# ielym/fastvision

Measured on AMD Instinct MI355X. Metric: images/sec (640×640, bs=32/GPU) YOLOv3 train step, 1/2/4/8 MI355X, higher is better.
Workload: dtype bf16

## Files before the change

### fastvision_amd/_lib.py

```python
import ctypes as C
import os

HERE = os.path.dirname(os.path.abspath(__file__))
LIB_PATH = os.path.join(HERE, 'csrc', 'libfastvision_amd.so')
if os.environ.get('FVA_LIB_PATH'):
    if os.environ.get('FVA_EXPERIMENTS') == '1':
        LIB_PATH = os.environ['FVA_LIB_PATH']
        import sys
        print(f'fastvision_amd: EXPERIMENT -- loading {LIB_PATH} instead of the in-tree library (FVA_LIB_PATH)', file=sys.stderr)
    else:
        raise RuntimeError('fastvision_amd: FVA_LIB_PATH is set but FVA_EXPERIMENTS=1 is not -- refusing to load another library silently')

F32, BF16 = 0, 1


class ConvDesc(C.Structure):
    _fields_ = [(n, C.c_int32) for n in ('dtype', 'B', 'H', 'W', 'Cin', 'Cout', 'ksize', 'stride', 'in_pad', 'dy_pad')]


class HeadLevel(C.Structure):
    _fields_ = [('data', C.c_void_p), ('grad', C.c_void_p),
                ('sb', C.c_int64), ('sa', C.c_int64), ('sy', C.c_int64), ('sx', C.c_int64), ('sk', C.c_int64),
                ('B', C.c_int32), ('A', C.c_int32), ('H', C.c_int32), ('W', C.c_int32), ('K', C.c_int32),
                ('anchor_w', C.c_float * 8), ('anchor_h', C.c_float * 8), ('stride', C.c_float)]
# ... 41 lines not shown

_P, _I, _L, _F = C.c_void_p, C.c_int32, C.c_int64, C.c_float
_D = C.POINTER(ConvDesc)
_H = C.POINTER(HeadLevel)

PROTOTYPES = {
    'fva_last_error': (C.c_char_p, []),
    'fva_version': (_I, []),
    'fva_profile_start': (_I, [_I]),
    'fva_profile_classes': (_I, [C.c_uint32, _I]),
    'fva_side_stream_fork': (_I, [_P, C.POINTER(C.c_void_p)]),
    'fva_side_stream_join': (_I, [_P]),
    'fva_side_stream_renew': (_I, []),
    'fva_conv_debug_stamps': (_I, [_P, _I]),
    'fva_conv_patch_kernel': (_I, [_I]),
    'fva_profile_stop': (_I, [_P, _P, _P, _I]),
    'fva_conv_pack_weights': (_I, [_D, _P, _P, _P, _P]),
    'fva_conv_packed_elems': (_L, [_D, _I]),
    'fva_conv_pack_weights_multi': (_I, [_P, _I, _L, _P]),
    'fva_conv_pack_weights_tiled': (_I, [_P, _I, _I, _P]),
    'fva_conv_last_kernel': (C.c_char_p, []),
    'fva_conv_fwd': (_I, [_D, _P, _P, _P, _P, _P]),
    'fva_conv1x1_fwd_apply': (_I, [_D, _P, _P, _P, _P, _I, _P, _P, _P, _P, _P]),
    'fva_conv_fwd_acc': (_I, [_D, _P, _P, _P, _P, _I, _P]),
    'fva_bn_acc_finalize': (_I, [C.POINTER(BnFwdAcc), _L, _I, _P]),
    'fva_bn_silu_apply_acc': (_I, [_I, _P, C.POINTER(BnFwdAcc), _P, _I, _P, _I, _I, _I, _I, _I, _P]),
    'fva_conv1x1_fwd_apply_acc': (_I, [_D, _P, C.POINTER(BnFwdAcc), _P, _I, _P, _P, _P, _P, _I, _P]),
    'fva_conv_fwd_bnact': (_I, [_D, _P, _P, _P, _P, _P, _P, _I, _P]),
    'fva_conv_stat_blocks': (_I, [_D]),
    'fva_conv_dgrad': (_I, [_D, _P, _P, _P, _P, _P]),
# ... 75 lines not shown
    'fva_softmax_ce_workspace': (_L, [_I]),
    'fva_softmax_ce': (_I, [_P, _P, _I, _P, _I, _I, _I, _P, _P, _P, _P]),
    'fva_top1_accuracy': (_I, [_P, _I, _P, _I, _I, _I, _P, _P, _P]),
    'fva_bn_relu_apply': (_I, [_I, _P, _P, _P, _P, _I, _I, _I, _I, _I, _P]),
    'fva_bn_relu_bwd_reduce': (_I, [_I, _P, _P, _P, _P, _P, _P, _P, _I, _L, _I, _P]),
    'fva_bn_relu_bwd_apply': (_I, [_I, _P, _P, _P, _P, _P, _P, _P, _P, _I, _I, _I, _I, _I, _P]),
    'fva_bn_bias_running_mean': (_I, [_I, _P, _P, _F, _P]),
    'fva_bn_eval_coeffs_bias': (_I, [_I, _P, _P, _P, _P, _P, _F, _P, _P, _P]),
    'fva_adaptive_avgpool7_fwd': (_I, [_I, _P, _I, _I, _I, _I, _I, _P, _P]),
    'fva_adaptive_avgpool7_bwd': (_I, [_I, _P, _I, _I, _I, _I, _P, _P]),
    'fva_dropout_fwd': (_I, [_I, _P, _P, _L, _F, _P, _P]),
    'fva_dropout_bwd': (_I, [_I, _P, _P, _P, _L, _F, _P]),
}
LABEL_I64, LABEL_F32 = 0, 1
REDUCE_MEAN, REDUCE_SUM = 0, 1
UNCHECKED = {'fva_conv_patch_kernel', 'fva_sgd_chunk_elems', 'fva_rows_relu_bwd_rows', 'fva_colour_workspace', 'fva_conv_dgrad_stat_rows', 'fva_bias_relu_bwd_rows', 'fva_colsum_scratch_rows', 'fva_last_error', 'fva_version', 'fva_profile_stop', 'fva_conv_last_kernel', 'fva_conv_packed_elems', 'fva_conv_stat_blocks', 'fva_conv_wgrad_workspace', 'fva_conv_wgrad_plan',
             'fva_stem_stat_blocks', 'fva_stem_fused_blocks', 'fva_stem_wgrad_workspace', 'fva_stem_fwd_workspace', 'fva_stem_wgrad_mfma_workspace', 'fva_bn_bwd_blocks', 'fva_bn_partial_rows', 'fva_yolov3_loss_workspace',
             'fva_demo_loss_workspace', 'fva_nms_candidates_workspace', 'fva_nms_select_workspace', 'fva_softmax_ce_workspace'}

_lib = None


def load():
    global _lib
    if _lib is not None:
        return _lib
    if not os.path.exists(LIB_PATH):
        raise RuntimeError(f'fastvision_amd: {LIB_PATH} is missing -- the HIP extension is REQUIRED (no CPU fallback). '
                           'Build it with `python fastvision_amd/csrc/build.py`.')
    lib = C.CDLL(LIB_PATH)
    for name, (res, args) in PROTOTYPES.items():
# ... 30 lines not shown
```

### fastvision_amd/csrc/conv_igemm.hip

```cpp
#include <stddef.h>
#include <stdlib.h>

#include "common.h"

namespace {

enum { EPI_STATS = 0, EPI_PLAIN = 1, EPI_HEAD = 2, EPI_BNACT = 3, EPI_BNB = 4 };
constexpr int MAX_TAPS = 10;

struct IgemmParams {
    const void* in;
    const void* wt;
    void* out;
    float* stats;
    int acc_rep, bnb_rep, ax_rep;
    long long* stats_acc;
    const float* bias;
    const float* scale;
    int act;
    const float* shift;
    int M, N, C;
    int OW, OHW;
    FastDiv div_ow, div_ohw;
    int in_img, in_row;
// ... 17 lines not shown
    const float *ax_scale, *ax_shift;
    int ax_pad, ax_res_pad, ax_H, ax_W;
    long long* ax_acc;
    long long* ax_zero;
    const float *ax_gamma, *ax_beta;
    float *ax_rm, *ax_rv;
    long long* ax_nbt;
    float ax_momentum, ax_eps;
    BnN ax_n;
    float *ax_save_mean, *ax_save_rstd, *ax_scale_out, *ax_shift_out;
    long long* stamps;
    int stamp_rows;
    int pt_tx, pt_ty, pt_H, pt_W;
    int pt_tiles, pt_tpb;
    FastDiv pt_div_tx, pt_div_img;
};

struct BnbCoef {
    float sc[8], sh[8], mu[8], rs[8];
};
__device__ __forceinline__ void bnb_load(const IgemmParams& p, int n, BnbCoef& k) {
#pragma unroll
    for (int e = 0; e < 8; ++e) {
        int c = n + e;
        c = c < p.N ? c : p.N - 1;
        c = c >= p.bnb_C ? c - p.bnb_C : c;
        k.sc[e] = p.bnb_scale[c]; k.sh[e] = p.bnb_shift[c]; k.mu[e] = p.bnb_mean[c]; k.rs[e] = p.bnb_rstd[c];
    }
}
template <int BN, int NT>
__device__ __forceinline__ float bnb_coef_at(const IgemmParams& p, int i, int n0) {
// ... 169 lines not shown
__device__ __forceinline__ void foreach_acc(Acc<float>& acc, int lane, F&& f) {
    const int r = lane & 31, h = lane >> 5;
#pragma unroll
    for (int mt = 0; mt < 2; ++mt)
#pragma unroll
        for (int nt = 0; nt < 2; ++nt)
#pragma unroll
            for (int e = 0; e < 16; ++e) f(mt * 32 + (e & 3) + 8 * (e >> 2) + 4 * h, nt * 32 + r, nt, acc.a[mt][nt][e]);
}

template <int N>
__device__ __forceinline__ void wait_vmcnt() {
    asm volatile("s_waitcnt vmcnt(%0)" ::"n"(N) : "memory");
}

template <typename T, int BM, int BN, int EPI, int NSTAGE, bool AX = false>
__global__ __launch_bounds__((BM / 64) * (BN / 64) * 64) void igemm_kernel(const IgemmParams p) {
    static_assert(!AX || (sizeof(T) == 2 && EPI == EPI_STATS), "the produced-operand form is the bf16 training forward of a 1x1 layer");
    constexpr int EPC = 16 / (int)sizeof(T);
    constexpr int BK = 8 * EPC;
    constexpr int WN = BN / 64;
    constexpr int NW = (BM / 64) * WN;
    constexpr int NT = NW * 64;
    static_assert(NW % 2 == 0, "the source swizzle assumes an even wave count");
    constexpr int A_BYTES = BM * 128, B_BYTES = BN * 128, STAGE = A_BYTES + B_BYTES;
    constexpr int A_ITERS = BM / (8 * NW), B_ITERS = BN / (8 * NW);
    constexpr bool IS_BF16 = sizeof(T) == 2;
    extern __shared__ __attribute__((aligned(16))) char smem[];

    const int tid = threadIdx.x, lane = tid & 63, w = tid >> 6;
    const int wr = w / WN, wc = w % WN;
    auto stamp = [&](int i) {
        if (p.stamps && tid == 0 && (int)blockIdx.x < p.stamp_rows) p.stamps[(int64_t)blockIdx.x * 8 + i] = wall_clock64();
    };
    stamp(0);

    const int nwg = gridDim.x, bid = blockIdx.x;
    const int xcd = bid & 7, xq = nwg >> 3, xr = nwg & 7;
    const int logical = (xcd < xr ? xcd * (xq + 1) : xr * (xq + 1) + (xcd - xr) * xq) + (bid >> 3);
    const int mblk = logical / p.nblocks, nblk = logical - mblk * p.nblocks;
    const int m0 = mblk * BM, n0 = nblk * BN;

    const T* a_ptr[A_ITERS];
    const T* b_ptr[B_ITERS];
    const int lrow = lane >> 3;
    const int sw = ((w & 1) << 2) + (lane >> 4);
    const int chunk = (lane & 7) ^ sw;
    const int tapsel = chunk >> 2;
    const int sub = p.halfrow ? (chunk & 3) : chunk;
#pragma unroll
    for (int i = 0; i < A_ITERS; ++i) {
        int m = m0 + (i * NW + w) * 8 + lrow;
        m = m < p.M ? m : p.M - 1;
        const uint32_t b = fd_div((uint32_t)m, p.div_ohw);
        const uint32_t rem = (uint32_t)m - b * (uint32_t)p.OHW;
        const uint32_t oy = fd_div(rem, p.div_ow);
// ... 7 lines not shown
        n = n < p.N ? n : p.N - 1;
        b_ptr[i] = (const T*)p.wt + (int64_t)n * p.C + sub * EPC;
    }

    constexpr bool USE_KTAB = BN >= 128;
    constexpr int COEF_BYTES = (EPI == EPI_BNB && IS_BF16 && BN >= 128) ? 4 * BN * 4 : 0;
    float* coef_tab = (float*)(smem + NSTAGE * STAGE);
    int* ktab = (int*)(smem + NSTAGE * STAGE + COEF_BYTES);
    constexpr int COEF_PER_THREAD = COEF_BYTES > 0 ? 4 * BN / NT : 0;
    float coef_v[COEF_PER_THREAD > 0 ? COEF_PER_THREAD : 1];
    if constexpr (COEF_BYTES > 0) {
#pragma unroll
        for (int j = 0; j < COEF_PER_THREAD; ++j) coef_v[j] = bnb_coef_at<BN, NT>(p, tid + j * NT, n0);
    }
    if constexpr (USE_KTAB) {
        const int nent = p.halfrow ? 2 * p.ktiles : p.ktiles;
        for (int e = tid; e < nent; e += NT) {
            int t, kk;
            if (p.halfrow) { t = e; kk = 0; }
            else if (p.ktaps) { kk = e / p.ktaps; t = e - kk * p.ktaps; }
            else { t = e / p.kt_per_tap; kk = e - t * p.kt_per_tap; }
            int tp = 0, tw = 0;
#pragma unroll
            for (int i = 0; i < MAX_TAPS; ++i)
                if (i == t) { tp = p.tap_pix[i]; tw = p.tap_w[i]; }
            ktab[2 * e] = tp * p.C + kk * BK;
            ktab[2 * e + 1] = tw * p.N * p.C + kk * BK;
        }
        __syncthreads();
    }
    stamp(6);
    int ld_tap = 0, ld_kk = 0;
    auto load_tile = [&](int kt, int stage) {
        char* sA = smem + stage * STAGE;
        char* sB = sA + A_BYTES;
        int aoff, boff;
        if constexpr (USE_KTAB) {
            const int e = p.halfrow ? 2 * kt + tapsel : kt;
            aoff = ktab[2 * e];
            boff = ktab[2 * e + 1];
// ... 22 lines not shown
        constexpr int CPR = BN / 8, RSTEP = NT / CPR;
        static_assert(BM * CPR / NT == 8, "the prefetch covers the whole store loop");
        const int cc = tid % CPR, r0 = tid / CPR;
        const int n = n0 + cc * 8;
#pragma unroll
        for (int j = 0; j < 8; ++j) {
            const int m = m0 + r0 + j * RSTEP;
            int64_t oi = 0;
            if (n < p.N && m < p.M) {
                int64_t pixel = m;
                if (!p.out_dense) {
                    const uint32_t b = fd_div((uint32_t)m, p.div_ohw);
                    const uint32_t rem = (uint32_t)m - b * (uint32_t)p.OHW;
                    const uint32_t oy = fd_div(rem, p.div_ow);
                    const uint32_t ox = rem - oy * (uint32_t)p.OW;
                    pixel = (int64_t)b * p.out_img + (int64_t)(oy * p.osy + p.ooy) * p.out_row + (ox * p.osx + p.oox);
                }
                oi = pixel * p.out_pitch + n;
            }
            if constexpr (EPI == EPI_BNB) y_pre[j] = ld_stream((const bf16_t*)p.bnb_y + oi);
            if (p.addend != nullptr) a_pre[j] = ld_stream((const bf16_t*)p.addend + oi);
        }
    }

    Acc<T> acc;
    if constexpr (sizeof(T) == 2) {
#pragma unroll
        for (int i = 0; i < 4; ++i)
#pragma unroll
            for (int j = 0; j < 4; ++j) acc.a[i][j] = f32x4{0.f, 0.f, 0.f, 0.f};
    } else {
// ... 147 lines not shown
            ax_fl[i] = (live ? 1u : 0u) | (zp > 0 && live ? ((ox == 0 ? 2u : 0u) | (ox == (uint32_t)p.ax_W - 1 ? 4u : 0u) | (oy == 0 ? 8u : 0u) |
                                                           (oy == (uint32_t)p.ax_H - 1 ? 16u : 0u)) : 0u);
        }
        ax_load_raw(0, std::integral_constant<int, 0>{});
        if constexpr (AXT) {
            for (int c = tid; c < p.C; c += NT) ax_coef(c, logical == 0, ax_tab[c], ax_tab[p.C + c]);
            __syncthreads();
        }
        if (AXT && p.ax_acc != nullptr && logical == 0) {
            if (tid == 0 && p.ax_nbt) *p.ax_nbt += 1;
            fx_zero(p.ax_zero, p.C, p.ax_rep, tid, NT);
        }
        ax_issue_b(0, 0);
    } else {
        load_tile(0, 0);
        if (p.ktiles > 1) load_tile(1, 1);
    }
    stamp(1);
    for (int kt = 0; kt < p.ktiles; ++kt) {
        if constexpr (AX) {
            if (AXS == 1 || (kt & 1) == 0) ax_step(kt, std::integral_constant<int, 0>{});
            else ax_step(kt, std::integral_constant<int, AXS - 1>{});
            if (kt == 0) stamp(2);
        } else {
        if (kt == 0 && p.ktiles > 1) wait_vmcnt<LPT>();
        else wait_vmcnt<0>();
        __builtin_amdgcn_s_barrier();
        if (kt == 0) stamp(2);
        if (kt >= 1 && kt + 1 < p.ktiles) load_tile(kt + 1, st_cur ^ 1);
        }
        const char* sA = smem + st_cur * STAGE;
        const char* sB = sA + A_BYTES;
        st_cur ^= 1;
        if constexpr (IS_BF16) {
            const int r = lane & 15, g = lane >> 4, sr = (r >> 1) & 7;
            const char* pa = sA + (wr * 64 + r) * 128;
            const char* pb = sB + (wc * 64 + r) * 128;
#pragma unroll
            for (int ks = 0; ks < 2; ++ks) {
                const int co = ((ks * 4 + g) ^ sr) << 4;
                bf16x8 af[4], bfr[4];
#pragma unroll
                for (int t = 0; t < 4; ++t) {
                    af[t] = *(const bf16x8*)(pa + t * 16 * 128 + co);
// ... 111 lines not shown
                        if (p.stats_acc != nullptr) fx_atomic_add(fx_replica(p.stats_acc, p.N, p.acc_rep), p.N, which, n0 + col, s);
                        else *(p.stats + ((int64_t)mblk * 2 + which) * p.N + n0 + col) = s;
                    }
                }
                __syncthreads();
            }
        }
    }

    auto out_pixel = [&](int m) -> int64_t {
        if (p.out_dense) return m;
        const uint32_t b = fd_div((uint32_t)m, p.div_ohw);
        const uint32_t rem = (uint32_t)m - b * (uint32_t)p.OHW;
        const uint32_t oy = fd_div(rem, p.div_ow);
        const uint32_t ox = rem - oy * (uint32_t)p.OW;
        return (int64_t)b * p.out_img + (int64_t)(oy * p.osy + p.ooy) * p.out_row + (ox * p.osx + p.oox);
    };

    if constexpr (EPI == EPI_HEAD) {
        float* out = (float*)p.out;
        foreach_acc(acc, lane, [&](int row, int col, int, float v) {
            const int m = m0 + wrow0 + row, n = n0 + wcol0 + col;
            if (m < p.M && n < p.N) out[(int64_t)m * p.out_pitch + n] = v + p.bias[n];
        });
    } else if constexpr (!IS_BF16) {
        float* out = (float*)p.out;
        int64_t pix_cache = -1;
        int m_cache = -1;
        constexpr bool bnb = EPI == EPI_BNB;
        float b1[2] = {0.f, 0.f}, b2[2] = {0.f, 0.f}, ksc[2], ksh[2], kmu[2], krs[2];
        if constexpr (bnb) {
// ... 38 lines not shown
                    if (lane < 32) {
                        red[(0 * WMc + wr) * BN + wcol0 + i * 32 + lane] = b1[i];
                        red[(1 * WMc + wr) * BN + wcol0 + i * 32 + lane] = b2[i];
                    }
                }
                __syncthreads();
                if (w < BN / 32) {
                    const int which = lane >> 5, col = w * 32 + (lane & 31);
                    float t = 0.f;
#pragma unroll
                    for (int k = 0; k < WMc; ++k) t += red[(which * WMc + k) * BN + col];
                    const int n = n0 + col;
                    const int sub = n >= p.bnb_C ? 1 : 0, per = p.N > p.bnb_C ? 2 : 1;
                    if (n < p.N) {
                        if (p.bnb_acc != nullptr) fx_atomic_add(fx_replica(p.bnb_acc, p.bnb_C, p.bnb_rep), p.bnb_C, which, n - sub * p.bnb_C, t);
                        else *(p.bnb_part + (((int64_t)(p.bnb_row0 + mblk) * per + sub) * 2 + which) * p.bnb_C + (n - sub * p.bnb_C)) = t;
                    }
                }
            }
        }
    } else {
        constexpr int PITCH = BN * 2 + 16;
        if constexpr (EPI == EPI_BNB && COEF_BYTES == 0) {
            coef_tab = (float*)(smem + BM * PITCH);
            static_assert(4 * BN <= NT || EPI != EPI_BNB || COEF_BYTES > 0, "one table entry per thread");
            if (tid < 4 * BN) coef_v[0] = bnb_coef_at<BN, NT>(p, tid, n0);
        }
        {
            const int r = lane & 15, g = lane >> 4;
#pragma unroll
            for (int mt = 0; mt < 4; ++mt)
// ... 1 lines not shown
                for (int nt = 0; nt < 4; ++nt) {
                    f32x4 v = acc.a[mt][nt];
                    const int col = wcol0 + nt * 16 + 4 * g;
                    if constexpr (EPI == EPI_BNACT) {
#pragma unroll
                        for (int j = 0; j < 4; ++j) v[j] = bnact_f(p, v[j], n0 + col + j < p.N ? n0 + col + j : p.N - 1);
                    }
                    *(u32x2*)(smem + (wrow0 + mt * 16 + r) * PITCH + col * 2) = u32x2{cvt_pk_bf16(v[0], v[1]), cvt_pk_bf16(v[2], v[3])};
                }
        }
        if constexpr (EPI == EPI_BNB && COEF_BYTES == 0) {
            if (tid < 4 * BN) coef_tab[tid] = coef_v[0];
        }
        __syncthreads();
        stamp(4);
        store_tile_bf16<EPI, BM, BN, NT, PITCH>(p, smem, tid, n0, mblk, [&](int row) { const int m = m0 + row; return m < p.M ? out_pixel(m) : (int64_t)-1; },
                                                EPI == EPI_BNB ? y_pre : nullptr, PREFETCH ? a_pre : nullptr, coef_tab);
    }
    if constexpr (AX) {

    }
    stamp(5);
}

template <typename T, int BM, int BN, int EPI, int NSTAGE, bool AX = false>
int launch_one(const IgemmParams& p, hipStream_t s) {
    const int mblocks = cdiv(p.M, BM);
    IgemmParams q = p;
    q.nblocks = cdiv(p.N, BN);
    static const bool stamp_tiles = [] { const char* e = getenv("FVA_STAMP_IGEMM"); return e && atoi(e) != 0; }();
    q.stamps = stamp_tiles ? fva_debug_stamps_ptr() : nullptr;
    q.stamp_rows = stamp_tiles ? fva_debug_stamps_rows() : 0;
    constexpr int KTAB_MAX = 16384;
    const int nent = (p.halfrow ? 2 : 1) * p.ktiles;
    if (BN >= 128 && nent * 8 > KTAB_MAX) return fva_fail(FVA_ERR_ARG, "igemm: %d k-tiles exceed the offset table (%d)", p.ktiles, KTAB_MAX / 8);
    const int ktab_bytes = BN >= 128 ? (nent * 8 > 4096 ? (nent * 8 + 255) & ~255 : 4096) : 0;
    constexpr int coef_bytes = (EPI == EPI_BNB && sizeof(T) == 2 && BN >= 128) ? 4 * BN * 4 : 0;
    const int smem = NSTAGE * (BM + BN) * 128 + ktab_bytes + coef_bytes;
    static bool attr_done = false;
    if (!attr_done) {
        (void)hipFuncSetAttribute((const void*)igemm_kernel<T, BM, BN, EPI, NSTAGE, AX>, hipFuncAttributeMaxDynamicSharedMemorySize,
                                  NSTAGE * (BM + BN) * 128 + (BN >= 128 ? KTAB_MAX : 0) + coef_bytes);
        attr_done = true;
    }
    hipLaunchKernelGGL((igemm_kernel<T, BM, BN, EPI, NSTAGE, AX>), dim3(mblocks * q.nblocks), dim3((BM / 64) * (BN / 64) * 64), smem, s, q);
    FVA_LAUNCH_CHECK("igemm_kernel");
    fva_note_kernel(AX ? (BM == 128 ? "igemm128ax" : "igemm256x64ax") : (BM == 128 ? "igemm128" : "igemm256x64"));
    return FVA_OK;
}

template <int CS, int BN, int NSL, int EPI>
__global__ __launch_bounds__(256, 2) void pconv_kernel(const IgemmParams p) {
    constexpr int TH = 8, TW = 32, PW = TW + 2, NPIX = (TH + 2) * PW;
    constexpr int PIXB = CS * 2;
    constexpr int CPP = PIXB / 16;
    constexpr int PPI = 1024 / PIXB;
    constexpr int PATCH_INSTR = (NPIX + PPI - 1) / PPI, PATCH_BYTES = PATCH_INSTR * 1024;
    constexpr int WSTEP_BYTES = BN * PIXB, WPW = WSTEP_BYTES / 1024 / 4;
    static_assert(WSTEP_BYTES % 4096 == 0, "whole DMA instructions per wave");
    constexpr int STEPS = 9 * NSL;
// ... 442 lines not shown
    p.pt_div_img = make_fastdiv(p.pt_tx * p.pt_ty);
    const int tiles = pdgrad2_tiles(B, H, W);
    if (p.C == 64 && p.N == 32) return launch_pdgrad2_one<64, 32, 1, EPI>(p, tiles, s);
    if (p.C == 128 && p.N == 64) return launch_pdgrad2_one<64, 64, 2, EPI>(p, tiles, s);
    return fva_fail(FVA_ERR_ARG, "pdgrad2: unsupported channels %d -> %d", p.C, p.N);
}

struct Igemm8Diag {
    long long* stamps;
    int stamp_rows;
};

#ifndef FVA_EPI_STAMPS
#define FVA_EPI_STAMPS 0
#endif
template <int EPI>
__global__ __launch_bounds__(512) void igemm8_kernel(const IgemmParams p, const Igemm8Diag sk) {
    constexpr int MT = 8;
    constexpr int WM = 16 * MT;
    constexpr int BM = 2 * WM, BN = 256, NT = 512, BK = 64;
    constexpr int HALF = 128 * 128, BUF = 4 * HALF;
    constexpr int EPI_BYTES = BM * (BN * 2 + 16);
    constexpr int TAB0 = EPI_BYTES > 2 * BUF ? EPI_BYTES : 2 * BUF;
    extern __shared__ __attribute__((aligned(16))) char smem[];
    const int tid = threadIdx.x, lane = tid & 63, w = tid >> 6;
    const int wr = w >> 2, wc = w & 3;
    auto stamp = [&](int i) {
        if (sk.stamps && tid == 0 && (int)blockIdx.x < sk.stamp_rows) {
            sk.stamps[(int64_t)blockIdx.x * 8 + i] = wall_clock64();
            sk.stamps[(int64_t)blockIdx.x * 8 + 4 + i] = clock64();
        }
    };
#if !FVA_EPI_STAMPS
    stamp(0);
#endif

    const int nwg = gridDim.x, bid = blockIdx.x;
    const int xcd = bid & 7, xq = nwg >> 3, xr = nwg & 7;
    const int logical = (xcd < xr ? xcd * (xq + 1) : xr * (xq + 1) + (xcd - xr) * xq) + (bid >> 3);
    const int KT = p.ktiles;

    int* ktab = (int*)(smem + TAB0);
    for (int e = tid; e < KT; e += NT) {
        int t, kk;
        if (p.ktaps) { kk = e / p.ktaps; t = e - kk * p.ktaps; }
        else { t = e / p.kt_per_tap; kk = e - t * p.kt_per_tap; }
        int tp = 0, tw = 0;
#pragma unroll
        for (int i = 0; i < MAX_TAPS; ++i)
            if (i == t) { tp = p.tap_pix[i]; tw = p.tap_w[i]; }
        ktab[2 * e] = tp * p.C + kk * BK;
        ktab[2 * e + 1] = tw * p.N * p.C + kk * BK;
    }

    const int lrow = lane >> 3;
    const int chunk = (lane & 7) ^ (((w & 1) << 2) + (lane >> 4));
    const int r = lane & 15, g = lane >> 4, sr = (r >> 1) & 7;
    const int co0 = (g ^ sr) << 4, co1 = ((4 + g) ^ sr) << 4;
    const int a_row = (wr * 64 + r) * 128, b_row = (wc * 32 + r) * 128;

    {
        const int tile = logical, kt0 = 0, kt1 = KT;
        const int mblk = tile / p.nblocks, nblk = tile - mblk * p.nblocks;
        const int m0 = mblk * BM, n0 = nblk * BN;
        __syncthreads();
        float* coef_tab = (float*)(smem + TAB0 + 4096);
        if constexpr (EPI == EPI_BNB) bnb_fill_lds<BN, NT>(p, coef_tab, tid, n0);

        uint32_t a_off[2][2], b_off[2][2];
#pragma unroll
        for (int h = 0; h < 2; ++h)
#pragma unroll
            for (int i = 0; i < 2; ++i) {
                const int rh = (i * 8 + w) * 8 + lrow;
                int m = m0 + (rh >> 6) * WM + h * 64 + (rh & 63);
                m = m < p.M ? m : p.M - 1;
                const uint32_t b = fd_div((uint32_t)m, p.div_ohw);
                const uint32_t rem = (uint32_t)m - b * (uint32_t)p.OHW;
                const uint32_t oy = fd_div(rem, p.div_ow);
// ... 154 lines not shown
                    if (n0 + col < p.N) {
                        if (p.stats_acc != nullptr) fx_atomic_add(fx_replica(p.stats_acc, p.N, p.acc_rep), p.N, which, n0 + col, s);
                        else *(p.stats + ((int64_t)mblk * 2 + which) * p.N + n0 + col) = s;
                    }
                }
                __syncthreads();
            }
        }

        auto out_pixel = [&](int m) -> int64_t {
            if (p.out_dense) return m;
            const uint32_t b = fd_div((uint32_t)m, p.div_ohw);
            const uint32_t rem = (uint32_t)m - b * (uint32_t)p.OHW;
            const uint32_t oy = fd_div(rem, p.div_ow);
            const uint32_t ox = rem - oy * (uint32_t)p.OW;
            return (int64_t)b * p.out_img + (int64_t)(oy * p.osy + p.ooy) * p.out_row + (ox * p.osx + p.oox);
        };
        constexpr int PITCH = BN * 2 + 16;
#if FVA_EPI_STAMPS
        stamp(1);
#endif
#pragma unroll
        for (int mi = 0; mi < MT; ++mi)
#pragma unroll
            for (int ni = 0; ni < 4; ++ni) {
                f32x4 v = acc[mi][ni];
                if constexpr (EPI == EPI_BNACT) {
#pragma unroll
                    for (int j = 0; j < 4; ++j) v[j] = bnact_f(p, v[j], n0 + col_e + ni * 16 + j);
                }
                *(u32x2*)(smem + (row_e + mi * 16) * PITCH + (col_e + ni * 16) * 2) = u32x2{cvt_pk_bf16(v[0], v[1]), cvt_pk_bf16(v[2], v[3])};
            }
        __syncthreads();
#if FVA_EPI_STAMPS
        stamp(2);
#endif
        store_tile_bf16<EPI, BM, BN, NT, PITCH>(p, smem, tid_e, n0, mblk, [&](int row) { const int m = m0 + row; return m < p.M ? out_pixel(m) : (int64_t)-1; },
                                                nullptr, nullptr, EPI == EPI_BNB ? coef_tab : nullptr);
    }
    stamp(3);
}

constexpr int IGEMM8_SMEM = 256 * (256 * 2 + 16) + 4096 + 4096;

inline bool igemm8_enabled() {
    static bool v = [] {
        const char* e = getenv("FVA_IGEMM8");
        return !e || atoi(e) != 0;
    }();
    return v;
}
inline bool use_igemm8(int dtype, int64_t M, int N, int C, int ntaps, int64_t in_pixels) {
    if (!igemm8_enabled() || dtype != FVA_BF16 || N % 256 || C % 64) return false;
    if (in_pixels * C * 2 >= (1ll << 31) || (int64_t)(ntaps + 1) * N * C * 2 >= (1ll << 31)) return false;
    const int64_t ktiles = (int64_t)ntaps * (C / 64), tiles = (int64_t)cdiv(M, 256) * (N / 256);
    if (ktiles > 496 || ktiles < 8) return false;
    if (tiles < 128) return false;
    static const int min_kt = [] { const char* e = getenv("FVA_IGEMM8_MINKT"); return e ? atoi(e) : 16; }();
    return ktiles >= min_kt || tiles <= 256;
}

long long* g_stamps = nullptr;
int g_stamp_rows = 0;

template <int EPI>
int launch_igemm8(const IgemmParams& p, hipStream_t s) {
    IgemmParams q = p;
    q.nblocks = p.N / 256;
    const int tiles = cdiv(p.M, 256) * q.nblocks;
    static bool attr_done = false;
    if (!attr_done) {
        (void)hipFuncSetAttribute((const void*)igemm8_kernel<EPI>, hipFuncAttributeMaxDynamicSharedMemorySize, IGEMM8_SMEM);
        attr_done = true;
    }
    Igemm8Diag sk{};
    sk.stamps = g_stamps;
    sk.stamp_rows = g_stamp_rows;
    hipLaunchKernelGGL((igemm8_kernel<EPI>), dim3(tiles), dim3(512), IGEMM8_SMEM, s, q, sk);
    fva_note_kernel("igemm8");
    FVA_LAUNCH_CHECK("igemm8_kernel");
    return FVA_OK;
}

inline bool wide_tile(int N) { return N >= 128; }

inline int tile_bm(int , int , int N) { return wide_tile(N) ? 128 : 256; }

template <int EPI>
int launch_igemm(int dtype, const IgemmParams& p, hipStream_t s) {
    if (dtype == FVA_BF16) {
        if constexpr (EPI != EPI_HEAD) {
            if (!p.halfrow && use_igemm8(dtype, p.M, p.N, p.C, p.ktiles / p.kt_per_tap, (int64_t)(p.M / p.OHW + 1) * p.in_img))
                return launch_igemm8<EPI>(p, s);
// ... 217 lines not shown
        }
    }
}

inline int pair_max_cin() {
    static int v = [] {
        const char* e = getenv("FVA_DGRAD_PAIR_MAX");
        return e ? atoi(e) : 64;
    }();
    return v;
}
inline bool dgrad_paired(int dtype, int ksize, int stride, int Cin, int Cout) {
    return ksize == 3 && stride == 2 && Cin <= pair_max_cin() && !use_pdgrad2(dtype, ksize, stride, Cout, Cin);
}

int packed_taps(const fva_conv_desc* d, int for_dgrad) {
    if (for_dgrad && dgrad_paired(d->dtype, d->ksize, d->stride, d->Cin, d->Cout)) return 12;

    const int kk = d->ksize * d->ksize;
    const int C = for_dgrad ? d->Cout : d->Cin;
    return (halfrow_mode(d->dtype, C) && (kk & 1)) ? kk + 1 : kk;
}

}

long long* fva_debug_stamps_ptr() { return g_stamps; }
int fva_debug_stamps_rows() { return g_stamp_rows; }
extern "C" {

int fva_conv_patch_kernel(int on) {
    const int prev = pconv_enabled() ? 1 : 0;
    g_pconv = on ? 1 : 0;
    return prev;
}

int fva_conv_debug_stamps(void* stamps, int32_t rows) {
    if (stamps && rows < 1) return fva_fail(FVA_ERR_ARG, "fva_conv_debug_stamps: rows must be >= 1");
    g_stamps = (long long*)stamps;
    g_stamp_rows = stamps ? rows : 0;
    return FVA_OK;
}

int64_t fva_conv_packed_elems(const fva_conv_desc* d, int for_dgrad) {
    if (!d) return 0;
    return (int64_t)packed_taps(d, for_dgrad) * d->Cout * d->Cin;
}

// ... 354 lines not shown
            if (rc) return rc;
            p.bnb_row0 += dgrad_launch_rows(d, p.M, p.N, p.C, nt, in_pixels);
        }
        return FVA_OK;
    }
    p.M = d->B * JH * JW;
    p.OW = JW;
    p.OHW = JH * JW;
    p.div_ow = make_fastdiv(p.OW);
    p.div_ohw = make_fastdiv(p.OHW);
    p.y0 = p.x0 = 0;
    p.out_dense = 0;
    p.out_img = d->H * d->W;
    p.out_row = d->W;
    p.osy = p.osx = 2;
    for (int py = 0; py < 2; ++py)
        for (int px = 0; px < 2; ++px) {
            int khs[2], yo[2], nky, kws[2], xo[2], nkx;
            if (py == 0) { nky = 1; khs[0] = 1; yo[0] = d->dy_pad; }
            else { nky = 2; khs[0] = 0; yo[0] = d->dy_pad + 1; khs[1] = 2; yo[1] = d->dy_pad; }
            if (px == 0) { nkx = 1; kws[0] = 1; xo[0] = d->dy_pad; }
            else { nkx = 2; kws[0] = 0; xo[0] = d->dy_pad + 1; kws[1] = 2; xo[1] = d->dy_pad; }
            int nt = 0;
            for (int a = 0; a < nky; ++a)
                for (int b = 0; b < nkx; ++b) {
                    p.tap_pix[nt] = yo[a] * p.in_row + xo[b];
                    p.tap_w[nt] = khs[a] * 3 + kws[b];
                    ++nt;
                }
            p.tap_w[nt] = 9;
            finish_taps(p, nt, d->dtype);
            p.ooy = py;
            p.oox = px;
            rc = f ? launch_igemm<EPI_BNB>(d->dtype, p, (hipStream_t)stream) : launch_igemm<EPI_PLAIN>(d->dtype, p, (hipStream_t)stream);
            if (rc) return rc;
            p.bnb_row0 += dgrad_launch_rows(d, p.M, p.N, p.C, nt, in_pixels);
        }
    return FVA_OK;
}

}
```

### include/fastvision_amd.h

```cpp
#ifndef FASTVISION_AMD_H
#define FASTVISION_AMD_H

#include <stdint.h>

#ifdef __cplusplus
extern "C" {
#endif

typedef enum { FVA_F32 = 0, FVA_BF16 = 1 } fva_dtype;

typedef enum {
    FVA_OK = 0,
    FVA_ERR_ARG = -1,
    FVA_ERR_LAUNCH = -2,
    FVA_ERR_WORKSPACE = -3
} fva_status;

const char* fva_last_error(void);
int fva_version(void);

int fva_profile_start(int32_t max_spans);
int fva_profile_classes(uint32_t mask, int32_t stride);

int fva_side_stream_fork(void* main_stream, void** side_stream);
// ... 15 lines not shown
typedef struct {
    const float* w;
    void* w_fwd;
    void* w_dgrad;
    int32_t Cout, Cin, ksize, taps_fwd, taps_dgrad, dtype;
    int32_t dgrad_paired;
    int32_t tile_start;
} fva_pack_entry;
int fva_conv_pack_weights_multi(const fva_pack_entry* table, int32_t n, int64_t max_elems, void* stream);
int fva_conv_pack_weights_tiled(const fva_pack_entry* table, int32_t n, int32_t total_tiles, void* stream);

const char* fva_conv_last_kernel(void);

int fva_conv_debug_stamps(void* stamps, int32_t rows);
int fva_conv_patch_kernel(int on);

int fva_conv_fwd(const fva_conv_desc* d, const void* x, const void* w_fwd, void* y, float* stats_partial, void* stream);
int fva_conv1x1_fwd_apply(const fva_conv_desc* d, const void* y_prev, const float* scale, const float* shift, const void* residual,
                          int32_t res_pad, void* z, const void* w_fwd, void* y, float* stats_partial, void* stream);
int fva_conv_fwd_bnact(const fva_conv_desc* d, const void* x, const void* w_fwd, const float* scale, const float* shift,
                       const void* residual, void* z, int32_t z_pad, void* stream);
int32_t fva_conv_stat_blocks(const fva_conv_desc* d);

int fva_conv_dgrad(const fva_conv_desc* d, const void* dy, const void* w_dgrad, void* dx, const void* addend, void* stream);

typedef struct {
    const void* y;
    const float *scale, *shift, *mean, *rstd;
    float* partial;
    int64_t* acc;
// ... 257 lines not shown
```

Baseline: 1123.

## Group the four stride-2 dgrad parity classes into single grouped GEMM launches

The stride-2 3x3 data-gradient conv used to run as four separate implicit-GEMM launches, one per output parity class, each with a different tap count. The classes are now packed into a per-launch table, and one grouped launch per kernel variant (igemm8 or the 128x128 tile) covers all of them, each block picking its class from its block index. This cuts launch count and the tail idle time between small launches. In exchange the params struct grows, blocks pay for class selection, and launches that mix 1-, 2- and 4-tap classes carry uneven per-block work. It is on by default and can be turned off with an env var or API toggle.

```diff
diff --git a/fastvision_amd/_lib.py b/fastvision_amd/_lib.py
--- a/fastvision_amd/_lib.py
+++ b/fastvision_amd/_lib.py
@@ -79,6 +79,7 @@
     'fva_side_stream_renew': (_I, []),
     'fva_conv_debug_stamps': (_I, [_P, _I]),
     'fva_conv_patch_kernel': (_I, [_I]),
+    'fva_conv_dgrad_grouped': (_I, [_I]),
     'fva_profile_stop': (_I, [_P, _P, _P, _I]),
     'fva_conv_pack_weights': (_I, [_D, _P, _P, _P, _P]),
     'fva_conv_packed_elems': (_L, [_D, _I]),
@@ -184,7 +185,7 @@
 }
 LABEL_I64, LABEL_F32 = 0, 1
 REDUCE_MEAN, REDUCE_SUM = 0, 1
-UNCHECKED = {'fva_conv_patch_kernel', 'fva_sgd_chunk_elems', 'fva_rows_relu_bwd_rows', 'fva_colour_workspace', 'fva_conv_dgrad_stat_rows', 'fva_bias_relu_bwd_rows', 'fva_colsum_scratch_rows', 'fva_last_error', 'fva_version', 'fva_profile_stop', 'fva_conv_last_kernel', 'fva_conv_packed_elems', 'fva_conv_stat_blocks', 'fva_conv_wgrad_workspace', 'fva_conv_wgrad_plan',
+UNCHECKED = {'fva_conv_patch_kernel', 'fva_conv_dgrad_grouped', 'fva_sgd_chunk_elems', 'fva_rows_relu_bwd_rows', 'fva_colour_workspace', 'fva_conv_dgrad_stat_rows', 'fva_bias_relu_bwd_rows', 'fva_colsum_scratch_rows', 'fva_last_error', 'fva_version', 'fva_profile_stop', 'fva_conv_last_kernel', 'fva_conv_packed_elems', 'fva_conv_stat_blocks', 'fva_conv_wgrad_workspace', 'fva_conv_wgrad_plan',
              'fva_stem_stat_blocks', 'fva_stem_fused_blocks', 'fva_stem_wgrad_workspace', 'fva_stem_fwd_workspace', 'fva_stem_wgrad_mfma_workspace', 'fva_bn_bwd_blocks', 'fva_bn_partial_rows', 'fva_yolov3_loss_workspace',
              'fva_demo_loss_workspace', 'fva_nms_candidates_workspace', 'fva_nms_select_workspace', 'fva_softmax_ce_workspace'}
 
diff --git a/fastvision_amd/csrc/conv_igemm.hip b/fastvision_amd/csrc/conv_igemm.hip
--- a/fastvision_amd/csrc/conv_igemm.hip
+++ b/fastvision_amd/csrc/conv_igemm.hip
@@ -7,6 +7,15 @@
 
 enum { EPI_STATS = 0, EPI_PLAIN = 1, EPI_HEAD = 2, EPI_BNACT = 3, EPI_BNB = 4 };
 constexpr int MAX_TAPS = 10;
+
+constexpr int GRP_CLASSES = 4, GRP_TAPS = 4;
+struct TapClass {
+    int tap_pix[GRP_TAPS], tap_w[GRP_TAPS];
+    int ntaps, ktiles;
+    int ooy, oox;
+    int bnb_row0;
+    int tile0;
+};
 
 struct IgemmParams {
     const void* in;
@@ -55,7 +64,23 @@
     int pt_tx, pt_ty, pt_H, pt_W;
     int pt_tiles, pt_tpb;
     FastDiv pt_div_tx, pt_div_img;
+    int ngrp, grp_tiles;
+    TapClass grp[GRP_CLASSES];
 };
+
+__device__ __forceinline__ TapClass grp_class(const IgemmParams& p, int logical) {
+    TapClass c = p.grp[0];
+#pragma unroll
+    for (int i = 1; i < GRP_CLASSES; ++i)
+        if (i < p.ngrp && logical >= p.grp[i].tile0) c = p.grp[i];
+    return c;
+}
+__device__ __forceinline__ void grp_tap(const TapClass& c, int t, int& tp, int& tw) {
+    tp = 0; tw = 0;
+#pragma unroll
+    for (int i = 0; i < GRP_TAPS; ++i)
+        if (i == t) { tp = c.tap_pix[i]; tw = c.tap_w[i]; }
+}
 
 struct BnbCoef {
     float sc[8], sh[8], mu[8], rs[8];
@@ -255,9 +280,10 @@
     asm volatile("s_waitcnt vmcnt(%0)" ::"n"(N) : "memory");
 }
 
-template <typename T, int BM, int BN, int EPI, int NSTAGE, bool AX = false>
+template <typename T, int BM, int BN, int EPI, int NSTAGE, bool AX = false, bool GRP = false>
 __global__ __launch_bounds__((BM / 64) * (BN / 64) * 64) void igemm_kernel(const IgemmParams p) {
     static_assert(!AX || (sizeof(T) == 2 && EPI == EPI_STATS), "the produced-operand form is the bf16 training forward of a 1x1 layer");
+    static_assert(!GRP || (!AX && BN >= 128 && (EPI == EPI_PLAIN || EPI == EPI_BNB)), "the grouped form is the stride-2 data gradient on the wide tile");
     constexpr int EPC = 16 / (int)sizeof(T);
     constexpr int BK = 8 * EPC;
     constexpr int WN = BN / 64;
@@ -276,11 +302,21 @@
     };
     stamp(0);
 
-    const int nwg = gridDim.x, bid = blockIdx.x;
+    int nwg = gridDim.x, bid = blockIdx.x;
+    TapClass cls = {};
+    if constexpr (GRP) {
+        cls = grp_class(p, bid);
+        bid -= cls.tile0;
+        nwg = p.grp_tiles;
+    }
     const int xcd = bid & 7, xq = nwg >> 3, xr = nwg & 7;
     const int logical = (xcd < xr ? xcd * (xq + 1) : xr * (xq + 1) + (xcd - xr) * xq) + (bid >> 3);
-    const int mblk = logical / p.nblocks, nblk = logical - mblk * p.nblocks;
+    const int tile = logical;
+    const int ktiles = GRP ? cls.ktiles : p.ktiles;
+    const int ooy = GRP ? cls.ooy : p.ooy, oox = GRP ? cls.oox : p.oox;
+    const int mblk = tile / p.nblocks, nblk = tile - mblk * p.nblocks;
     const int m0 = mblk * BM, n0 = nblk * BN;
+    const int srow = GRP ? cls.bnb_row0 + mblk : mblk;
 
     const T* a_ptr[A_ITERS];
     const T* b_ptr[B_ITERS];
@@ -318,16 +354,21 @@
         for (int j = 0; j < COEF_PER_THREAD; ++j) coef_v[j] = bnb_coef_at<BN, NT>(p, tid + j * NT, n0);
     }
     if constexpr (USE_KTAB) {
-        const int nent = p.halfrow ? 2 * p.ktiles : p.ktiles;
+        const int nent = (!GRP && p.halfrow) ? 2 * ktiles : ktiles;
+        const int ktaps = GRP ? (p.ktaps ? cls.ntaps : 0) : p.ktaps;
         for (int e = tid; e < nent; e += NT) {
             int t, kk;
-            if (p.halfrow) { t = e; kk = 0; }
-            else if (p.ktaps) { kk = e / p.ktaps; t = e - kk * p.ktaps; }
+            if (!GRP && p.halfrow) { t = e; kk = 0; }
+            else if (ktaps) { kk = e / ktaps; t = e - kk * ktaps; }
             else { t = e / p.kt_per_tap; kk = e - t * p.kt_per_tap; }
             int tp = 0, tw = 0;
-#pragma unroll
-            for (int i = 0; i < MAX_TAPS; ++i)
-                if (i == t) { tp = p.tap_pix[i]; tw = p.tap_w[i]; }
+            if constexpr (GRP) {
+                grp_tap(cls, t, tp, tw);
+            } else {
+#pragma unroll
+                for (int i = 0; i < MAX_TAPS; ++i)
+                    if (i == t) { tp = p.tap_pix[i]; tw = p.tap_w[i]; }
+            }
             ktab[2 * e] = tp * p.C + kk * BK;
             ktab[2 * e + 1] = tw * p.N * p.C + kk * BK;
         }
@@ -380,7 +421,7 @@
                     const uint32_t rem = (uint32_t)m - b * (uint32_t)p.OHW;
                     const uint32_t oy = fd_div(rem, p.div_ow);
                     const uint32_t ox = rem - oy * (uint32_t)p.OW;
-                    pixel = (int64_t)b * p.out_img + (int64_t)(oy * p.osy + p.ooy) * p.out_row + (ox * p.osx + p.oox);
+                    pixel = (int64_t)b * p.out_img + (int64_t)(oy * p.osy + ooy) * p.out_row + (ox * p.osx + oox);
                 }
                 oi = pixel * p.out_pitch + n;
             }
@@ -558,20 +599,20 @@
         ax_issue_b(0, 0);
     } else {
         load_tile(0, 0);
-        if (p.ktiles > 1) load_tile(1, 1);
+        if (ktiles > 1) load_tile(1, 1);
     }
     stamp(1);
-    for (int kt = 0; kt < p.ktiles; ++kt) {
+    for (int kt = 0; kt < ktiles; ++kt) {
         if constexpr (AX) {
             if (AXS == 1 || (kt & 1) == 0) ax_step(kt, std::integral_constant<int, 0>{});
             else ax_step(kt, std::integral_constant<int, AXS - 1>{});
             if (kt == 0) stamp(2);
         } else {
-        if (kt == 0 && p.ktiles > 1) wait_vmcnt<LPT>();
+        if (kt == 0 && ktiles > 1) wait_vmcnt<LPT>();
         else wait_vmcnt<0>();
         __builtin_amdgcn_s_barrier();
         if (kt == 0) stamp(2);
-        if (kt >= 1 && kt + 1 < p.ktiles) load_tile(kt + 1, st_cur ^ 1);
+        if (kt >= 1 && kt + 1 < ktiles) load_tile(kt + 1, st_cur ^ 1);
         }
         const char* sA = smem + st_cur * STAGE;
         const char* sB = sA + A_BYTES;
@@ -713,7 +754,7 @@
         const uint32_t rem = (uint32_t)m - b * (uint32_t)p.OHW;
         const uint32_t oy = fd_div(rem, p.div_ow);
         const uint32_t ox = rem - oy * (uint32_t)p.OW;
-        return (int64_t)b * p.out_img + (int64_t)(oy * p.osy + p.ooy) * p.out_row + (ox * p.osx + p.oox);
+        return (int64_t)b * p.out_img + (int64_t)(oy * p.osy + ooy) * p.out_row + (ox * p.osx + oox);
     };
 
     if constexpr (EPI == EPI_HEAD) {
@@ -782,7 +823,7 @@
                     const int sub = n >= p.bnb_C ? 1 : 0, per = p.N > p.bnb_C ? 2 : 1;
                     if (n < p.N) {
                         if (p.bnb_acc != nullptr) fx_atomic_add(fx_replica(p.bnb_acc, p.bnb_C, p.bnb_rep), p.bnb_C, which, n - sub * p.bnb_C, t);
-                        else *(p.bnb_part + (((int64_t)(p.bnb_row0 + mblk) * per + sub) * 2 + which) * p.bnb_C + (n - sub * p.bnb_C)) = t;
+                        else *(p.bnb_part + (((int64_t)(p.bnb_row0 + srow) * per + sub) * 2 + which) * p.bnb_C + (n - sub * p.bnb_C)) = t;
                     }
                 }
             }
@@ -814,7 +855,7 @@
         }
         __syncthreads();
         stamp(4);
-        store_tile_bf16<EPI, BM, BN, NT, PITCH>(p, smem, tid, n0, mblk, [&](int row) { const int m = m0 + row; return m < p.M ? out_pixel(m) : (int64_t)-1; },
+        store_tile_bf16<EPI, BM, BN, NT, PITCH>(p, smem, tid, n0, srow, [&](int row) { const int m = m0 + row; return m < p.M ? out_pixel(m) : (int64_t)-1; },
                                                 EPI == EPI_BNB ? y_pre : nullptr, PREFETCH ? a_pre : nullptr, coef_tab);
     }
     if constexpr (AX) {
@@ -823,9 +864,9 @@
     stamp(5);
 }
 
-template <typename T, int BM, int BN, int EPI, int NSTAGE, bool AX = false>
+template <typename T, int BM, int BN, int EPI, int NSTAGE, bool AX = false, bool GRP = false>
 int launch_one(const IgemmParams& p, hipStream_t s) {
-    const int mblocks = cdiv(p.M, BM);
+    const int mblocks = cdiv(p.M, BM) * (GRP ? p.ngrp : 1);
     IgemmParams q = p;
     q.nblocks = cdiv(p.N, BN);
     static const bool stamp_tiles = [] { const char* e = getenv("FVA_STAMP_IGEMM"); return e && atoi(e) != 0; }();
@@ -839,11 +880,11 @@
     const int smem = NSTAGE * (BM + BN) * 128 + ktab_bytes + coef_bytes;
     static bool attr_done = false;
     if (!attr_done) {
-        (void)hipFuncSetAttribute((const void*)igemm_kernel<T, BM, BN, EPI, NSTAGE, AX>, hipFuncAttributeMaxDynamicSharedMemorySize,
+        (void)hipFuncSetAttribute((const void*)igemm_kernel<T, BM, BN, EPI, NSTAGE, AX, GRP>, hipFuncAttributeMaxDynamicSharedMemorySize,
                                   NSTAGE * (BM + BN) * 128 + (BN >= 128 ? KTAB_MAX : 0) + coef_bytes);
         attr_done = true;
     }
-    hipLaunchKernelGGL((igemm_kernel<T, BM, BN, EPI, NSTAGE, AX>), dim3(mblocks * q.nblocks), dim3((BM / 64) * (BN / 64) * 64), smem, s, q);
+    hipLaunchKernelGGL((igemm_kernel<T, BM, BN, EPI, NSTAGE, AX, GRP>), dim3(mblocks * q.nblocks), dim3((BM / 64) * (BN / 64) * 64), smem, s, q);
     FVA_LAUNCH_CHECK("igemm_kernel");
     fva_note_kernel(AX ? (BM == 128 ? "igemm128ax" : "igemm256x64ax") : (BM == 128 ? "igemm128" : "igemm256x64"));
     return FVA_OK;
@@ -1316,8 +1357,9 @@
 #ifndef FVA_EPI_STAMPS
 #define FVA_EPI_STAMPS 0
 #endif
-template <int EPI>
+template <int EPI, bool GRP = false>
 __global__ __launch_bounds__(512) void igemm8_kernel(const IgemmParams p, const Igemm8Diag sk) {
+    static_assert(!GRP || EPI == EPI_PLAIN || EPI == EPI_BNB, "the grouped form is the stride-2 data gradient");
     constexpr int MT = 8;
     constexpr int WM = 16 * MT;
     constexpr int BM = 2 * WM, BN = 256, NT = 512, BK = 64;
@@ -1337,20 +1379,32 @@
     stamp(0);
 #endif
 
-    const int nwg = gridDim.x, bid = blockIdx.x;
+    int nwg = gridDim.x, bid = blockIdx.x;
+    TapClass cls = {};
+    if constexpr (GRP) {
+        cls = grp_class(p, bid);
+        bid -= cls.tile0;
+        nwg = p.grp_tiles;
+    }
     const int xcd = bid & 7, xq = nwg >> 3, xr = nwg & 7;
     const int logical = (xcd < xr ? xcd * (xq + 1) : xr * (xq + 1) + (xcd - xr) * xq) + (bid >> 3);
-    const int KT = p.ktiles;
+    const int KT = GRP ? cls.ktiles : p.ktiles;
+    const int ktaps = GRP ? (p.ktaps ? cls.ntaps : 0) : p.ktaps;
+    const int ooy = GRP ? cls.ooy : p.ooy, oox = GRP ? cls.oox : p.oox;
 
     int* ktab = (int*)(smem + TAB0);
     for (int e = tid; e < KT; e += NT) {
         int t, kk;
-        if (p.ktaps) { kk = e / p.ktaps; t = e - kk * p.ktaps; }
+        if (ktaps) { kk = e / ktaps; t = e - kk * ktaps; }
         else { t = e / p.kt_per_tap; kk = e - t * p.kt_per_tap; }
         int tp = 0, tw = 0;
-#pragma unroll
-        for (int i = 0; i < MAX_TAPS; ++i)
-            if (i == t) { tp = p.tap_pix[i]; tw = p.tap_w[i]; }
+        if constexpr (GRP) {
+            grp_tap(cls, t, tp, tw);
+        } else {
+#pragma unroll
+            for (int i = 0; i < MAX_TAPS; ++i)
+                if (i == t) { tp = p.tap_pix[i]; tw = p.tap_w[i]; }
+        }
         ktab[2 * e] = tp * p.C + kk * BK;
         ktab[2 * e + 1] = tw * p.N * p.C + kk * BK;
     }
@@ -1365,6 +1419,7 @@
         const int tile = logical, kt0 = 0, kt1 = KT;
         const int mblk = tile / p.nblocks, nblk = tile - mblk * p.nblocks;
         const int m0 = mblk * BM, n0 = nblk * BN;
+        const int srow = GRP ? cls.bnb_row0 + mblk : mblk;
         __syncthreads();
         float* coef_tab = (float*)(smem + TAB0 + 4096);
         if constexpr (EPI == EPI_BNB) bnb_fill_lds<BN, NT>(p, coef_tab, tid, n0);
@@ -1549,7 +1604,7 @@
             const uint32_t rem = (uint32_t)m - b * (uint32_t)p.OHW;
             const uint32_t oy = fd_div(rem, p.div_ow);
             const uint32_t ox = rem - oy * (uint32_t)p.OW;
-            return (int64_t)b * p.out_img + (int64_t)(oy * p.osy + p.ooy) * p.out_row + (ox * p.osx + p.oox);
+            return (int64_t)b * p.out_img + (int64_t)(oy * p.osy + ooy) * p.out_row + (ox * p.osx + oox);
         };
         constexpr int PITCH = BN * 2 + 16;
 #if FVA_EPI_STAMPS
@@ -1570,7 +1625,7 @@
 #if FVA_EPI_STAMPS
         stamp(2);
 #endif
-        store_tile_bf16<EPI, BM, BN, NT, PITCH>(p, smem, tid_e, n0, mblk, [&](int row) { const int m = m0 + row; return m < p.M ? out_pixel(m) : (int64_t)-1; },
+        store_tile_bf16<EPI, BM, BN, NT, PITCH>(p, smem, tid_e, n0, srow, [&](int row) { const int m = m0 + row; return m < p.M ? out_pixel(m) : (int64_t)-1; },
                                                 nullptr, nullptr, EPI == EPI_BNB ? coef_tab : nullptr);
     }
     stamp(3);
@@ -1598,20 +1653,20 @@
 long long* g_stamps = nullptr;
 int g_stamp_rows = 0;
 
-template <int EPI>
+template <int EPI, bool GRP = false>
 int launch_igemm8(const IgemmParams& p, hipStream_t s) {
     IgemmParams q = p;
     q.nblocks = p.N / 256;
-    const int tiles = cdiv(p.M, 256) * q.nblocks;
+    const int tiles = cdiv(p.M, 256) * q.nblocks * (GRP ? p.ngrp : 1);
     static bool attr_done = false;
     if (!attr_done) {
-        (void)hipFuncSetAttribute((const void*)igemm8_kernel<EPI>, hipFuncAttributeMaxDynamicSharedMemorySize, IGEMM8_SMEM);
+        (void)hipFuncSetAttribute((const void*)igemm8_kernel<EPI, GRP>, hipFuncAttributeMaxDynamicSharedMemorySize, IGEMM8_SMEM);
         attr_done = true;
     }
     Igemm8Diag sk{};
     sk.stamps = g_stamps;
     sk.stamp_rows = g_stamp_rows;
-    hipLaunchKernelGGL((igemm8_kernel<EPI>), dim3(tiles), dim3(512), IGEMM8_SMEM, s, q, sk);
+    hipLaunchKernelGGL((igemm8_kernel<EPI, GRP>), dim3(tiles), dim3(512), IGEMM8_SMEM, s, q, sk);
     fva_note_kernel("igemm8");
     FVA_LAUNCH_CHECK("igemm8_kernel");
     return FVA_OK;
@@ -1859,6 +1914,15 @@
     return ksize == 3 && stride == 2 && Cin <= pair_max_cin() && !use_pdgrad2(dtype, ksize, stride, Cout, Cin);
 }
 
+int g_dgrad_group = -1;
+inline bool dgrad_group_enabled() {
+    if (g_dgrad_group < 0) {
+        const char* e = getenv("FVA_DGRAD_GROUP");
+        g_dgrad_group = (!e || atoi(e) != 0) ? 1 : 0;
+    }
+    return g_dgrad_group != 0;
+}
+
 int packed_taps(const fva_conv_desc* d, int for_dgrad) {
     if (for_dgrad && dgrad_paired(d->dtype, d->ksize, d->stride, d->Cin, d->Cout)) return 12;
 
@@ -1876,6 +1940,12 @@
 int fva_conv_patch_kernel(int on) {
     const int prev = pconv_enabled() ? 1 : 0;
     g_pconv = on ? 1 : 0;
+    return prev;
+}
+
+int fva_conv_dgrad_grouped(int on) {
+    const int prev = dgrad_group_enabled() ? 1 : 0;
+    g_dgrad_group = on ? 1 : 0;
     return prev;
 }
 
@@ -2260,6 +2330,10 @@
     p.out_img = d->H * d->W;
     p.out_row = d->W;
     p.osy = p.osx = 2;
+    TapClass cls[4];
+    bool k8[4];
+    const bool halfrow = halfrow_mode(d->dtype, p.C);
+    int row0 = 0;
     for (int py = 0; py < 2; ++py)
         for (int px = 0; px < 2; ++px) {
             int khs[2], yo[2], nky, kws[2], xo[2], nkx;
@@ -2267,21 +2341,67 @@
             else { nky = 2; khs[0] = 0; yo[0] = d->dy_pad + 1; khs[1] = 2; yo[1] = d->dy_pad; }
             if (px == 0) { nkx = 1; kws[0] = 1; xo[0] = d->dy_pad; }
             else { nkx = 2; kws[0] = 0; xo[0] = d->dy_pad + 1; kws[1] = 2; xo[1] = d->dy_pad; }
+            TapClass& c = cls[py * 2 + px];
+            c = TapClass();
             int nt = 0;
             for (int a = 0; a < nky; ++a)
                 for (int b = 0; b < nkx; ++b) {
-                    p.tap_pix[nt] = yo[a] * p.in_row + xo[b];
-                    p.tap_w[nt] = khs[a] * 3 + kws[b];
+                    c.tap_pix[nt] = yo[a] * p.in_row + xo[b];
+                    c.tap_w[nt] = khs[a] * 3 + kws[b];
                     ++nt;
                 }
-            p.tap_w[nt] = 9;
-            finish_taps(p, nt, d->dtype);
-            p.ooy = py;
-            p.oox = px;
-            rc = f ? launch_igemm<EPI_BNB>(d->dtype, p, (hipStream_t)stream) : launch_igemm<EPI_PLAIN>(d->dtype, p, (hipStream_t)stream);
+            c.ntaps = nt;
+            c.ooy = py;
+            c.oox = px;
+            c.bnb_row0 = row0;
+            k8[py * 2 + px] = !halfrow && use_igemm8(d->dtype, p.M, p.N, p.C, nt, in_pixels);
+            row0 += dgrad_launch_rows(d, p.M, p.N, p.C, nt, in_pixels);
+        }
+    auto launch_class = [&](const TapClass& c) {
+        IgemmParams q = p;
+        for (int t = 0; t < c.ntaps; ++t) { q.tap_pix[t] = c.tap_pix[t]; q.tap_w[t] = c.tap_w[t]; }
+        q.tap_w[c.ntaps] = 9;
+        finish_taps(q, c.ntaps, d->dtype);
+        q.ooy = c.ooy;
+        q.oox = c.oox;
+        q.bnb_row0 = c.bnb_row0;
+        return f ? launch_igemm<EPI_BNB>(d->dtype, q, (hipStream_t)stream) : launch_igemm<EPI_PLAIN>(d->dtype, q, (hipStream_t)stream);
+    };
+    if (!dgrad_group_enabled() || halfrow || !wide_tile(p.N)) {
+        for (int i = 0; i < 4; ++i) {
+            rc = launch_class(cls[i]);
             if (rc) return rc;
-            p.bnb_row0 += dgrad_launch_rows(d, p.M, p.N, p.C, nt, in_pixels);
-        }
+        }
+        return FVA_OK;
+    }
+    static const int order[4] = {3, 2, 1, 0};
+    for (int kind = 1; kind >= 0; --kind) {
+        IgemmParams q = p;
+        int n = 0, maxt = 0;
+        for (int j = 0; j < 4; ++j)
+            if (k8[order[j]] == (kind == 1)) {
+                q.grp[n++] = cls[order[j]];
+                maxt = cls[order[j]].ntaps > maxt ? cls[order[j]].ntaps : maxt;
+            }
+        if (n == 0) continue;
+        if (n == 1) {
+            rc = launch_class(q.grp[0]);
+            if (rc) return rc;
+            continue;
+        }
+        finish_taps(q, maxt, d->dtype);
+        const int tiles = kind == 1 ? cdiv(q.M, 256) * (q.N / 256) : cdiv(q.M, 128) * cdiv(q.N, 128);
+        for (int j = 0; j < n; ++j) {
+            q.grp[j].ktiles = q.grp[j].ntaps * q.kt_per_tap;
+            q.grp[j].tile0 = j * tiles;
+        }
+        q.ngrp = n;
+        q.grp_tiles = tiles;
+        if (kind == 1) rc = f ? launch_igemm8<EPI_BNB, true>(q, (hipStream_t)stream) : launch_igemm8<EPI_PLAIN, true>(q, (hipStream_t)stream);
+        else if (d->dtype == FVA_BF16) rc = f ? launch_one<bf16_t, 128, 128, EPI_BNB, 2, false, true>(q, (hipStream_t)stream) : launch_one<bf16_t, 128, 128, EPI_PLAIN, 2, false, true>(q, (hipStream_t)stream);
+        else rc = f ? launch_one<float, 128, 128, EPI_BNB, 2, false, true>(q, (hipStream_t)stream) : launch_one<float, 128, 128, EPI_PLAIN, 2, false, true>(q, (hipStream_t)stream);
+        if (rc) return rc;
+    }
     return FVA_OK;
 }
 
diff --git a/include/fastvision_amd.h b/include/fastvision_amd.h
--- a/include/fastvision_amd.h
+++ b/include/fastvision_amd.h
@@ -53,6 +53,7 @@
 
 int fva_conv_debug_stamps(void* stamps, int32_t rows);
 int fva_conv_patch_kernel(int on);
+int fva_conv_dgrad_grouped(int on);
 
 int fva_conv_fwd(const fva_conv_desc* d, const void* x, const void* w_fwd, void* y, float* stats_partial, void* stream);
 int fva_conv1x1_fwd_apply(const fva_conv_desc* d, const void* y_prev, const float* scale, const float* shift, const void* residual,
```

Result: no change. 1129, median of 6 (+0.5%).
